# lichunshang/vision-enhanced-lidar-odometry

Measured on AMD Instinct MI355X. Metric: scan-pairs/sec + achieved HBM GB/s, 120k-pt HDL-64E frame-to-frame ICP, higher is better.
Workload: dtype f32 association / f64 residuals+solve

## Files before the change

vision-enhanced-lidar-odometry_amd/csrc/velo_kernels.h:

```cpp
#pragma once
#include <hip/hip_runtime.h>
#include <stdint.h>

#include "velo_device_math.h"

#ifndef VELO_DEF_LOAD
#define VELO_DEF_LOAD 0
#endif
#ifndef VELO_DEF_ASSOC
#define VELO_DEF_ASSOC 0
#endif
#ifndef VELO_DEF_LMA
#define VELO_DEF_LMA 0
#endif
#ifndef VELO_DEF_LMB
#define VELO_DEF_LMB 0
#endif

namespace velo {

constexpr int kWave = 64;
constexpr int kNumAcc = 28;
constexpr int kEvalThreads = 256;
constexpr int kMaxEvalBlocks = 512;
// ... 1042 lines not shown
                        const float d2 = dist2_f(qx, qy, qz, sp.x, sp.y, sp.z);
                        const unsigned long long key = ((unsigned long long)__float_as_uint(d2) << 32) | (unsigned)__float_as_int(sp.w);
                        if (key < b2) {
                            const int ring = G.sring[j];
                            if (key < b1) {
                                if (ring != b1ring) b2 = b1;
                                b1 = key; b1ring = ring;
                            } else if (ring != b1ring) {
                                b2 = key;
                            }
                        }
                    }
                }
            }
        }
    }
    if (active) finish_correspondence(qi, psrc, qx, qy, qz, b1, b2, key_inf, tgt, tgt_off, ring_of, norm_cond, out, want_aux != 0);
}
#else
;
#endif

struct Top2 {
    unsigned long long b1, b2;
    int b1ring, b2ring;
    float b2d;
};
__device__ __forceinline__ void top2_update(Top2& t, unsigned long long key, int ring) {
    if (key < t.b2) {
        if (key < t.b1) {
            if (ring != t.b1ring) { t.b2 = t.b1; t.b2ring = t.b1ring; }
            t.b1 = key; t.b1ring = ring;
        } else if (ring != t.b1ring) {
            t.b2 = key; t.b2ring = ring;
        }
        t.b2d = __uint_as_float((unsigned)(t.b2 >> 32));
    }
}

__device__ __forceinline__ int wave_min_i(int v) {
#pragma unroll
    for (int off = 32; off > 0; off >>= 1) v = min(v, __shfl_xor(v, off));
    return v;
}
__device__ __forceinline__ int wave_max_i(int v) {
#pragma unroll
    for (int off = 32; off > 0; off >>= 1) v = max(v, __shfl_xor(v, off));
    return v;
}

#ifndef VELO_ASSOC_SYNC_LEAN
#define VELO_ASSOC_SYNC_LEAN 1
#endif
constexpr int kTileCap = 512;
typedef float f32x2 __attribute__((ext_vector_type(2)));

template <int NW, int MINW, bool DBG>
__global__ void __launch_bounds__(NW * 64, MINW)
assoc_search_v3_kernel(PoseScalars P, GridView G, const float4* __restrict__ src, const int* __restrict__ q_src, int q_begin, int q_end,
                       const float4* __restrict__ tgt, const int* __restrict__ tgt_off, const int* __restrict__ ring_of,
                       unsigned gate_bits, double norm_cond, int cluster_w, float h_safe, AssocOut out, int want_aux, int dbg, int xcd_map) {
    constexpr int NT = NW * 64;
    constexpr int NRUN = 2 * NT;
    __shared__ float4 s_xy[kTileCap / 2];
    __shared__ float4 s_zg[kTileCap / 2];
    __shared__ int s_ring[kTileCap];
    __shared__ int s_run_j0[NRUN];
    __shared__ int s_run_off[NRUN + 1];
    __shared__ int s_wave_tot[NW];
    __shared__ unsigned long long m1[NW][64], m2[NW][64];
    __shared__ int mr[NW][64];

    const int tid = threadIdx.x;
    const int lane = tid & 63;
    const int wid = __builtin_amdgcn_readfirstlane(tid >> 6);
    long long tacc[8] = {0, 0, 0, 0, 0, 0, 0, 0};
    long long tlast = (DBG && (dbg & 8)) ? (long long)__builtin_readcyclecounter() : 0;
#define VELO_STAMP(k) do { if (DBG && (dbg & 8)) { const long long now__ = (long long)__builtin_readcyclecounter(); tacc[k] += now__ - tlast; tlast = now__; } } while (0)
    const int n_groups = (q_end - q_begin + 63) >> 6;
    const int per_xcd = (n_groups + 7) >> 3;
    const int group = xcd_map ? (int)(blockIdx.x & 7) * per_xcd + (int)(blockIdx.x >> 3) : (int)blockIdx.x;
    if (group >= n_groups || (xcd_map && (int)(blockIdx.x >> 3) >= per_xcd)) return;
    if ((DBG && (dbg & 32)) && threadIdx.x == 0) out.wg_times[2 * group] = __builtin_amdgcn_s_memrealtime();
    const int qi = q_begin + group * 64 + lane;
    const bool active = qi < q_end;
    const unsigned long long key_inf = ((unsigned long long)gate_bits + 1ull) << 32;
    float qx = 0.f, qy = 0.f, qz = 0.f;
    Top2 t;
    t.b1 = key_inf; t.b2 = key_inf; t.b1ring = -1; t.b2ring = -1; t.b2d = __uint_as_float(gate_bits + 1u);
    const GridDesc g = G.d;
    int cx = 0, cy = 0, cz = 0;
    if (active) {
        const float4 psrc = src[q_src[qi]];
        transform_query(P, psrc, &qx, &qy, &qz);
        cx = cell_coord(qx, g.ox, g.inv_h, g.nx); cy = cell_coord(qy, g.oy, g.inv_h, g.ny); cz = cell_coord(qz, g.oz, g.inv_h, g.nz);
    }
    VELO_STAMP(0);
    const f32x2 qx2 = {qx, qx}, qy2 = {qy, qy}, qz2 = {qz, qz};
    float* s_xy_f = reinterpret_cast<float*>(s_xy);
    float* s_zg_f = reinterpret_cast<float*>(s_zg);
    bool pending = active;
    for (;;) {
        const unsigned long long pm = __ballot(pending);
        if (pm == 0ull) break;
        const int leader = (int)__ffsll((long long)pm) - 1;
        const int scx = __builtin_amdgcn_readlane(cx, leader), scy = __builtin_amdgcn_readlane(cy, leader), scz = __builtin_amdgcn_readlane(cz, leader);
// ... 129 lines not shown
                m1[wid][lane] = t.b1; m2[wid][lane] = t.b2; mr[wid][lane] = t.b1ring;
                __syncthreads();
#pragma unroll
                for (int w = 0; w < NW; w++) {
                    if (w == wid) continue;
                    const unsigned long long c1 = m1[w][lane], c2 = m2[w][lane];
                    if (c1 < t.b2) top2_update(t, c1, mr[w][lane]);
                    if (c2 < t.b2) top2_update(t, c2, ring_of[(int)(unsigned)(c2 & 0xffffffffull) - out.first_point]);
                }
                __syncthreads();
            }
            const float rw = __uint_as_float((unsigned)__builtin_amdgcn_readfirstlane(wave_max_i(member ? (int)__float_as_uint(t.b2d) : 0)));
            const float reach = (float)e * h_safe;
            VELO_STAMP(6);
            if (reach * reach > rw) break;
            e_prev = e;
            e = max(e + 1, (int)ceilf(sqrtf(rw) / h_safe));
            if ((float)e * h_safe * ((float)e * h_safe) <= rw) e++;
        }
        pending = pending && !member;
    }
    if (NW > 1 && wid != 0) return;
    if (active) finish_correspondence(qi, src[q_src[qi]], qx, qy, qz, t.b1, t.b2, key_inf, tgt, tgt_off, ring_of, norm_cond, out, want_aux != 0);
    VELO_STAMP(7);
    if ((DBG && (dbg & 32)) && tid == 0) out.wg_times[2 * group + 1] = __builtin_amdgcn_s_memrealtime();
    if ((DBG && (dbg & 8)) && tid == 0) { for (int k = 0; k < 8; k++) atomicAdd((unsigned long long*)&out.dbg[k], (unsigned long long)tacc[k]); }
#undef VELO_STAMP
}

struct CellBox { int x0, x1, y0, y1, z0, z1; };
__device__ __forceinline__ CellBox query_box(const GridDesc& g, float qx, float qy, float qz, int cx, int cy, int cz, float r, bool clip) {
    asm volatile("" : "+v"(r));
    CellBox b;
    b.x0 = cell_coord(qx - r, g.ox, g.inv_h, g.nx); b.x1 = cell_coord(qx + r, g.ox, g.inv_h, g.nx);
    b.y0 = cell_coord(qy - r, g.oy, g.inv_h, g.ny); b.y1 = cell_coord(qy + r, g.oy, g.inv_h, g.ny);
    b.z0 = cell_coord(qz - r, g.oz, g.inv_h, g.nz); b.z1 = cell_coord(qz + r, g.oz, g.inv_h, g.nz);
    if (clip) {
        b.x0 = max(b.x0, cx - 1); b.x1 = min(b.x1, cx + 1);
        b.y0 = max(b.y0, cy - 1); b.y1 = min(b.y1, cy + 1);
        b.z0 = max(b.z0, cz - 1); b.z1 = min(b.z1, cz + 1);
    }
    return b;
}

__device__ __forceinline__ void top2_merge_xor(Top2& t, int mask) {
    const unsigned long long o1 = __shfl_xor(t.b1, mask), o2 = __shfl_xor(t.b2, mask);
    const int r1 = __shfl_xor(t.b1ring, mask), r2 = __shfl_xor(t.b2ring, mask);
    if (o1 < t.b2) top2_update(t, o1, r1);
    if (o2 < t.b2) top2_update(t, o2, r2);
}

#define kXcdChunks (reinterpret_cast<const int*>(8))
#define kXcdTiles (reinterpret_cast<const int*>(16))
template <int NW, int MINW, bool DBG, int PPT, int ASKER>
__device__ __forceinline__ void
assoc_search_v5_body(const PoseScalars& P_in, const PoseRecord* __restrict__ P_dev, int* __restrict__ chain_fail, const GridView& G, const float4* __restrict__ qpts, int q_begin, int q_end,
                     const float4* __restrict__ tgt_pad, const int* __restrict__ tgt_off,
                     unsigned gate_bits, double norm_cond, int cluster_w, float h_safe, const AssocOut& out, int want_aux, const int* __restrict__ group_perm, int dbg, int asker_rows,
                     const int block_x) {
    constexpr int NT = NW * 64;
    constexpr int NRUN = 2 * NT;
    static_assert(kTileCap % (2 * PPT) == 0, "the tile must hold whole trips (the padding of the last trip stays inside it)");
    __shared__ float4 s_xy[kTileCap / 2];
    __shared__ float4 s_zg[kTileCap / 2];
    __shared__ int s_ring[kTileCap];
    __shared__ int s_run_j0[NRUN];
    __shared__ int s_run_off[NRUN + 1];
    __shared__ int s_wave_tot[NW];
    __shared__ int s_lo[NT], s_hi[NT], s_plo[NT], s_phi[NT];
    __shared__ int s_box[2][6][64];
    __shared__ int s_phase[9];
    __shared__ float s_q[3][64];
#define VELO_Q(x, y, z) const float x = s_q[0][lane], y = s_q[1][lane], z = s_q[2][lane]
    static_assert(NW * 64 * 16 <= (int)sizeof(float4) * (kTileCap / 2) && NW * 64 * 8 <= (int)sizeof(int) * kTileCap, "merge scratch must fit the tile");
    unsigned long long (*m1)[64] = reinterpret_cast<unsigned long long (*)[64]>(s_xy);
    unsigned long long (*m2)[64] = m1 + NW;
    int (*mr)[64] = reinterpret_cast<int (*)[64]>(s_ring);
    int (*mr2)[64] = mr + NW;

    const int tid = threadIdx.x;
    const int lane = tid & 63;
    const int wid = __builtin_amdgcn_readfirstlane(tid >> 6);
    constexpr int lead = 0;
    if (chain_fail && *chain_fail) return;
    if (P_dev && !P_dev->ready) { if (block_x == 0 && tid == 0) *chain_fail = 1; return; }
    const PoseScalars& P = P_dev ? P_dev->P : P_in;
    long long tacc[8] = {0, 0, 0, 0, 0, 0, 0, 0};
    long long tlast = (DBG && (dbg & 8)) ? (long long)__builtin_readcyclecounter() : 0;
#define VELO_STAMP(k) do { if (DBG && (dbg & 8)) { const long long now__ = (long long)__builtin_readcyclecounter(); tacc[k] += now__ - tlast; tlast = now__; } } while (0)
    int group = (int)block_x;
    if (group_perm == kXcdChunks) {
        const int n_groups = (q_end - q_begin + 63) / 64, per = (n_groups + 7) / 8;
        group = (block_x & 7) * per + (block_x >> 3);
        if (group >= n_groups) return;
    } else if (group_perm == kXcdTiles) {
        const int n_groups = (q_end - q_begin + 63) / 64, per = (n_groups + 63) / 64;
        const int k = block_x & 7, j = block_x >> 3, b = j / per, w = j - b * per;
        group = (b * 8 + ((k + 8 - (b & 7)) & 7)) * per + w;
        if (b >= 8 || group >= n_groups) return;
    } else if (group_perm) group = group_perm[block_x];
    if (out.n_valid_next && block_x == 0 && tid == 0) *out.n_valid_next = 0;
    if (ASKER == 2 && block_x == 0 && tid == 0) *out.ask_count_next = 0;
    if (DBG && out.wg_times && tid == 0) out.wg_times[2 * group] = __builtin_amdgcn_s_memrealtime();
    const int qi = q_begin + group * 64 + lane;
    const bool active = qi < q_end;
    const unsigned long long key_inf = ((unsigned long long)gate_bits + 1ull) << 32;
    Top2 t;
    t.b1 = key_inf; t.b2 = key_inf; t.b1ring = -1; t.b2ring = -1; t.b2d = __uint_as_float(gate_bits + 1u);
    const GridDesc g = G.d;
#if VELO_ASSOC_SYNC_LEAN
    {
        float qx = 0.f, qy = 0.f, qz = 0.f;
        if (active) {
            const float4 psrc = qpts[qi];
            const bool seeded = out.prev_a && !(DBG && (dbg & 512));
            float4 sa = make_float4(0.f, 0.f, 0.f, __int_as_float(-1)), sb = sa;
            int2 sr = make_int2(-1, -1);
            if (seeded) { sa = out.prev_a[qi]; sb = out.prev_b[qi]; sr = out.prev_r[qi]; }
            transform_query(P, psrc, &qx, &qy, &qz);
            if (__float_as_int(sa.w) >= 0) {
                const float d = dist2_f(sa.x, sa.y, sa.z, qx, qy, qz);
                if (__float_as_uint(d) <= gate_bits) top2_update(t, ((unsigned long long)__float_as_uint(d) << 32) | (unsigned)(__float_as_int(sa.w) + out.first_point), sr.x);
            }
            if (__float_as_int(sb.w) >= 0) {
                const float d = dist2_f(sb.x, sb.y, sb.z, qx, qy, qz);
                if (__float_as_uint(d) <= gate_bits) top2_update(t, ((unsigned long long)__float_as_uint(d) << 32) | (unsigned)(__float_as_int(sb.w) + out.first_point), sr.y);
            }
        }
        s_q[0][lane] = qx; s_q[1][lane] = qy; s_q[2][lane] = qz;
        s_lo[tid] = 1 << 28; s_hi[tid] = -(1 << 28); s_plo[tid] = 1 << 28; s_phi[tid] = -(1 << 28);
    }
#else
    {
        unsigned long long* sb = reinterpret_cast<unsigned long long*>(s_zg);
        int* sr = s_ring;
        if (wid == lead) {
            float qx = 0.f, qy = 0.f, qz = 0.f;
            if (active) {
                const float4 psrc = qpts[qi];
                const bool seeded = out.prev_a && !(DBG && (dbg & 512));
                float4 sa = make_float4(0.f, 0.f, 0.f, __int_as_float(-1)), sb = sa;
                int2 sr = make_int2(-1, -1);
                if (seeded) { sa = out.prev_a[qi]; sb = out.prev_b[qi]; sr = out.prev_r[qi]; }
                transform_query(P, psrc, &qx, &qy, &qz);
                if (__float_as_int(sa.w) >= 0) {
                    const float d = dist2_f(sa.x, sa.y, sa.z, qx, qy, qz);
                    if (__float_as_uint(d) <= gate_bits) top2_update(t, ((unsigned long long)__float_as_uint(d) << 32) | (unsigned)(__float_as_int(sa.w) + out.first_point), sr.x);
                }
                if (__float_as_int(sb.w) >= 0) {
                    const float d = dist2_f(sb.x, sb.y, sb.z, qx, qy, qz);
                    if (__float_as_uint(d) <= gate_bits) top2_update(t, ((unsigned long long)__float_as_uint(d) << 32) | (unsigned)(__float_as_int(sb.w) + out.first_point), sr.y);
                }
            }
            s_q[0][lane] = qx; s_q[1][lane] = qy; s_q[2][lane] = qz;
            sb[lane] = t.b1; sb[64 + lane] = t.b2; sr[lane] = t.b1ring; sr[64 + lane] = t.b2ring;
        }
        __syncthreads();
        if (wid != lead) {
            t.b1 = sb[lane]; t.b2 = sb[64 + lane]; t.b1ring = sr[lane]; t.b2ring = sr[64 + lane];
            t.b2d = __uint_as_float((unsigned)(t.b2 >> 32));
        }
        __syncthreads();
    }
#endif
    VELO_STAMP(0);
    float* s_xy_f = reinterpret_cast<float*>(s_xy);
    float* s_zg_f = reinterpret_cast<float*>(s_zg);
    const int big = 1 << 28;
    bool pending = active;
    bool deferred = false;
    unsigned long long gstat[6] = {0, 0, 0, 0, 0, 0};
    for (;;) {
        const unsigned long long pm = __ballot(pending);
        if (pm == 0ull) break;
        const int leader = (int)__ffsll((long long)pm) - 1;
        bool member;
        {
            VELO_Q(qx, qy, qz);
            int cx = 0, cy = 0, cz = 0;
            if (active) { cx = cell_coord(qx, g.ox, g.inv_h, g.nx); cy = cell_coord(qy, g.oy, g.inv_h, g.ny); cz = cell_coord(qz, g.oz, g.inv_h, g.nz); }
            const int scx = __builtin_amdgcn_readlane(cx, leader), scy = __builtin_amdgcn_readlane(cy, leader), scz = __builtin_amdgcn_readlane(cz, leader);
            member = pending && abs(cx - scx) <= cluster_w && abs(cy - scy) <= cluster_w && abs(cz - scz) <= cluster_w;
        }
        if (DBG && (dbg & 16) && tid == 0) atomicAdd(&out.dbg[0], 1ull);
        if (DBG && (dbg & 32)) gstat[0]++;
        const float r1 = sqrtf(t.b2d) * 1.0001f + 1e-6f;
        bool asker_phase = false;
        const int dense_rows = (ASKER && !DBG) ? (dbg & 0xfffff) : 0, dense_far = (ASKER && !DBG) ? (dbg >> 20) : 0;
        bool asker_all = false;
        for (int ph = 0; ph < 2; ph++) {
            if (ph == 1 && s_phase[7] == 0) break;
            if (wid == lead) {
                bool asks0 = member;
                CellBox bb;
                int rows_all = 0;
                VELO_Q(qx, qy, qz);
                const int cx = cell_coord(qx, g.ox, g.inv_h, g.nx), cy = cell_coord(qy, g.oy, g.inv_h, g.ny), cz = cell_coord(qz, g.oz, g.inv_h, g.nz);
                if (ph == 0) bb = query_box(g, qx, qy, qz, cx, cy, cz, r1, true);
                else {
                    const float rq = sqrtf(t.b2d) * 1.0001f + 1e-6f;
                    bb = query_box(g, qx, qy, qz, cx, cy, cz, rq, false);
                    asks0 = member && !(bb.x0 >= s_box[0][0][lane] && bb.x1 <= s_box[0][1][lane] && bb.y0 >= s_box[0][2][lane] &&
                                        bb.y1 <= s_box[0][3][lane] && bb.z0 >= s_box[0][4][lane] && bb.z1 <= s_box[0][5][lane]);
                    rows_all = asks0 ? (bb.y1 - bb.y0 + 1) * (bb.z1 - bb.z0 + 1) : 0;
#pragma unroll
                    for (int off = 32; off > 0; off >>= 1) rows_all += __shfl_xor(rows_all, off);
                }
                s_box[ph][0][lane] = bb.x0; s_box[ph][1][lane] = bb.x1; s_box[ph][2][lane] = bb.y0;
                s_box[ph][3][lane] = bb.y1; s_box[ph][4][lane] = bb.z0; s_box[ph][5][lane] = bb.z1;
                const unsigned long long am0 = __ballot(asks0);
                const unsigned long long far0 = (ph == 0) ? __ballot(member && r1 > h_safe) : 1ull;
                const unsigned long long far4 = (ASKER && ph == 0) ? __ballot(member && r1 > 4.0f * h_safe) : 0ull;
                const int y0 = wave_min_i(asks0 ? bb.y0 : big), y1 = wave_max_i(asks0 ? bb.y1 : -big);
                const int z0 = wave_min_i(asks0 ? bb.z0 : big), z1 = wave_max_i(asks0 ? bb.z1 : -big);
                if (lane == 0) {
                    s_phase[0] = max(y0, 0); s_phase[1] = min(y1, g.ny - 1); s_phase[2] = max(z0, 0); s_phase[3] = min(z1, g.nz - 1);
                    s_phase[4] = (int)(unsigned)(am0 & 0xffffffffull); s_phase[5] = (int)(unsigned)(am0 >> 32); s_phase[6] = rows_all;
                    if (ph == 0) s_phase[7] = (int)__popcll(far0);
                    if (ASKER && ph == 0) s_phase[8] = (int)__popcll(far4);
                }
            }
            __syncthreads();
            if (ASKER && ph == 0 && dense_rows > 0) {
                const int ny0 = s_phase[1] - s_phase[0] + 1, nz0 = s_phase[3] - s_phase[2] + 1;
// ... 92 lines not shown
                if (tid == 0) s_run_off[NRUN] = total;
                __syncthreads();
                VELO_STAMP(2);
                if (DBG && (dbg & 2)) total = 0;
                if (DBG && (dbg & 32)) { gstat[1]++; gstat[2] += (unsigned long long)total; }
                if (DBG && (dbg & 16) && tid == 0) { atomicAdd(&out.dbg[1], 1ull); atomicAdd(&out.dbg[2], (unsigned long long)total); if (ph == 1) atomicAdd(&out.dbg[3], (unsigned long long)total); atomicAdd(&out.dbg[4], (unsigned long long)nrows); }
                for (int tbase = 0; tbase < total; tbase += kTileCap) {
                    const int tn = min(total - tbase, kTileCap);
                    const int tn2 = (tn + 2 * PPT - 1) / (2 * PPT) * (2 * PPT);
                    for (int i = tid; i < tn2; i += NT) {
                        float4 c = make_float4(__builtin_inff(), __builtin_inff(), __builtin_inff(), __int_as_float(0x7fffffff));
                        int cr = 0x7fffffff;
                        if (i < tn) {
                            const int slot = tbase + i;
                            int lo = 0;
#pragma unroll
                            for (int step = NRUN / 2; step > 0; step >>= 1) {
                                if (s_run_off[lo + step] <= slot) lo += step;
                            }
                            const int j = s_run_j0[lo] + (slot - s_run_off[lo]);
                            c = G.sorted[j];
                            cr = G.sring[j];
                        }
                        const int pr = i >> 1, hb = i & 1;
                        s_xy_f[4 * pr + hb] = c.x; s_xy_f[4 * pr + 2 + hb] = c.y;
                        s_zg_f[4 * pr + hb] = c.z; s_zg_f[4 * pr + 2 + hb] = c.w;
                        s_ring[i] = cr;
                    }
                    __syncthreads();
                    VELO_STAMP(3);
                    const int npairs = tn2 >> 1;
                    if (member && !(DBG && (dbg & 1))) {
                        const int2* s_ring2 = reinterpret_cast<const int2*>(s_ring);
                        for (int pi = wid * PPT; pi < npairs; pi += NW * PPT) {
                            float4 a[PPT], bq[PPT];
                            int2 rg[PPT];
#pragma unroll
                            for (int u = 0; u < PPT; u++) { a[u] = s_xy[pi + u]; bq[u] = s_zg[pi + u]; rg[u] = s_ring2[pi + u]; }
                            float d2x[PPT], d2y[PPT];
                            {
                                VELO_Q(qx, qy, qz);
#pragma unroll
                                for (int u = 0; u < PPT; u++) {
                                    d2x[u] = dist2_f(qx, qy, qz, a[u].x, a[u].z, bq[u].x);
                                    d2y[u] = dist2_f(qx, qy, qz, a[u].y, a[u].w, bq[u].y);
                                }
                            }
                            float dmin = fminf(d2x[0], d2y[0]);
#pragma unroll
                            for (int u = 1; u < PPT; u++) dmin = fminf(dmin, fminf(d2x[u], d2y[u]));
                            if (dmin <= t.b2d) {
#pragma unroll
                                for (int u = 0; u < PPT; u++) {
                                    if (d2x[u] <= t.b2d) {
                                        const unsigned long long key = ((unsigned long long)__float_as_uint(d2x[u]) << 32) | (unsigned)__float_as_int(bq[u].z);
                                        top2_update(t, key, rg[u].x);
                                    }
                                    if (d2y[u] <= t.b2d) {
                                        const unsigned long long key = ((unsigned long long)__float_as_uint(d2y[u]) << 32) | (unsigned)__float_as_int(bq[u].w);
                                        top2_update(t, key, rg[u].y);
                                    }
                                }
                            }
                        }
                    }
                    VELO_STAMP(4);
                    __syncthreads();
                    VELO_STAMP(5);
                }
            }
            if (NW > 1) {
                m1[wid][lane] = t.b1; m2[wid][lane] = t.b2; mr[wid][lane] = t.b1ring; mr2[wid][lane] = t.b2ring;
                __syncthreads();
#pragma unroll
                for (int w = 0; w < NW; w++) {
                    if (w == wid) continue;
                    const unsigned long long c1 = m1[w][lane], c2 = m2[w][lane];
                    if (c1 < t.b2) top2_update(t, c1, mr[w][lane]);
                    if (c2 < t.b2) top2_update(t, c2, mr2[w][lane]);
                }
                if (!VELO_ASSOC_SYNC_LEAN || ASKER != 0) __syncthreads();
            }
            VELO_STAMP(6);
        }
        if (ASKER == 2 && asker_phase) {
            VELO_Q(qx, qy, qz);
            const int cx = cell_coord(qx, g.ox, g.inv_h, g.nx), cy = cell_coord(qy, g.oy, g.inv_h, g.ny), cz = cell_coord(qz, g.oz, g.inv_h, g.nz);
            const float rq0 = sqrtf(t.b2d) * 1.0001f + 1e-6f;
            const CellBox b2 = query_box(g, qx, qy, qz, cx, cy, cz, rq0, false);
            const bool asks = member && (asker_all || !(b2.x0 >= s_box[0][0][lane] && b2.x1 <= s_box[0][1][lane] && b2.y0 >= s_box[0][2][lane] &&
                                                        b2.y1 <= s_box[0][3][lane] && b2.z0 >= s_box[0][4][lane] && b2.z1 <= s_box[0][5][lane]));
            if (wid == 0) {
                const unsigned long long am = __ballot(asks);
                int base = 0;
                if (lane == 0 && am != 0ull) base = atomicAdd(out.ask_count, (int)__popcll(am));
                base = __builtin_amdgcn_readfirstlane(base);
                if (asks) {
                    const int q_of_lane = q_begin + group * 64 + lane;
                    out.ask_list[base + (int)__popcll(am & ((1ull << lane) - 1ull))] = q_of_lane;
                    out.ask_keys[2 * (size_t)q_of_lane] = t.b1; out.ask_keys[2 * (size_t)q_of_lane + 1] = t.b2;
                    out.ask_rings[q_of_lane] = make_int2(t.b1ring, t.b2ring);
                }
            }
            deferred = deferred || asks;
        } else if (ASKER == 1 && asker_phase) {
            const float cap = 4.0f * h_safe;
// ... 37 lines not shown
                    const int nrows_a = (on && x0 <= x1 && ny > 0 && nz > 0) ? ny * nz : 0;
                    const float rcp_ny = 1.0f / (float)max(ny, 1);
                    for (int r0 = 0; r0 < nrows_a; r0 += LPA) {
                        const int r = r0 + sl;
                        int j0 = 0, len = 0;
                        if (r < nrows_a) {
                            int zq = (int)((float)r * rcp_ny), yr = r - zq * ny;
                            if (yr < 0) { zq--; yr += ny; } else if (yr >= ny) { zq++; yr -= ny; }
                            const int row = ((z0 + zq) * g.ny + (y0 + yr));
                            j0 = grid_start(G, row, x0); len = grid_start(G, row, x1 + 1) - j0;
                        }
                        int inc = len;
#pragma unroll
                        for (int off = 1; off < LPA; off <<= 1) { const int v = __shfl_up(inc, off, LPA); if (sl >= off) inc += v; }
                        const int total = __shfl(inc, LPA - 1, LPA);
                        w_j0[sl] = j0; w_off[sl] = inc - len;
                        if (sl == 0) w_off[LPA] = total;
                        __builtin_amdgcn_fence(__ATOMIC_RELEASE, "wavefront");
                        __builtin_amdgcn_wave_barrier();
                        __builtin_amdgcn_fence(__ATOMIC_ACQUIRE, "wavefront");
                        if (DBG && (dbg & 32)) gstat[4] += (unsigned long long)total;
                        if (DBG && (dbg & 16) && sl == 0) { atomicAdd(&out.dbg[2], (unsigned long long)total); atomicAdd(&out.dbg[3], (unsigned long long)total); atomicAdd(&out.dbg[4], (unsigned long long)min(LPA, nrows_a - r0)); }
                        for (int slot = sl; slot < total; slot += LPA) {
                            int lo = 0;
#pragma unroll
                            for (int step = LPA / 2; step > 0; step >>= 1) { if (w_off[lo + step] <= slot) lo += step; }
                            const int j = w_j0[lo] + (slot - w_off[lo]);
                            const float4 c = G.sorted[j];
                            const float d = dist2_f(ax, ay, az, c.x, c.y, c.z);
                            if (d <= tl.b2d) top2_update(tl, ((unsigned long long)__float_as_uint(d) << 32) | (unsigned)__float_as_int(c.w), G.sring[j]);
                        }
                        __builtin_amdgcn_fence(__ATOMIC_RELEASE, "wavefront");
                        __builtin_amdgcn_wave_barrier();
                        __builtin_amdgcn_fence(__ATOMIC_ACQUIRE, "wavefront");
                    }
#pragma unroll
                    for (int m = 1; m < LPA; m <<= 1) top2_merge_xor(tl, m);
                    if (on && sl == 0) { m1[0][la] = tl.b1; m2[0][la] = tl.b2; mr[0][la] = tl.b1ring; mr2[0][la] = tl.b2ring; }
                }
                __syncthreads();
                if (asks) {
                    t.b1 = m1[0][lane]; t.b2 = m2[0][lane]; t.b1ring = mr[0][lane]; t.b2ring = mr2[0][lane];
                    t.b2d = __uint_as_float((unsigned)(t.b2 >> 32));
                }
                __syncthreads();
            }
            if (DBG && (dbg & 32)) gstat[5] += __builtin_amdgcn_s_memrealtime() - t_ask0;
            }
            VELO_STAMP(6);
        }
        pending = pending && !member;
        if (VELO_ASSOC_SYNC_LEAN && ASKER == 0 && __ballot(pending) != 0ull) __syncthreads();
    }
    if (NW > 1 && wid != lead) return;
    VELO_Q(qx, qy, qz);
    int lane_fin = lane;
    asm volatile("" : "+v"(lane_fin));
    const int qi_fin = q_begin + group * 64 + lane_fin;
    const bool active_fin = qi_fin < q_end;
#define qi qi_fin
#define active active_fin
    if (DBG && (dbg & 128)) {
        if (active) { out.p[qi] = make_float4(qx, qy, qz, 0.f); out.n[qi] = make_float4((float)(t.b1 >> 32), (float)(t.b2 >> 32), 0.f, 0.f); out.v0[qi] = make_float4(0.f, 0.f, 0.f, 0.f); }
    } else
    if (active && !deferred) finish_correspondence_pad(qi, qpts, qx, qy, qz, t.b1, t.b2, t.b1ring, t.b2ring, key_inf, tgt_pad, tgt_off, norm_cond, out, want_aux != 0);
    VELO_STAMP(7);
    if (DBG && out.wg_times && tid == 0) {
        out.wg_times[2 * group + 1] = __builtin_amdgcn_s_memrealtime();
        const int n_groups = (q_end - q_begin + 63) / 64;
        for (int k = 0; k < 6; k++) out.wg_times[2 * (size_t)n_groups + 14 * (size_t)group + k] = gstat[k];
        for (int k = 0; k < 8; k++) out.wg_times[2 * (size_t)n_groups + 14 * (size_t)group + 6 + k] = (unsigned long long)tacc[k];
    }
    if (DBG && (dbg & 8) && tid == 0) { for (int k = 0; k < 8; k++) atomicAdd((unsigned long long*)&out.dbg[k], (unsigned long long)tacc[k]); }
#undef VELO_STAMP
#undef VELO_Q
#undef qi
#undef active
}


template <int NW, int MINW, bool DBG, int PPT, int ASKER>
__global__ void __launch_bounds__(NW * 64, MINW)
assoc_search_v5_kernel(PoseScalars P, const PoseRecord* __restrict__ P_dev, int* __restrict__ chain_fail, GridView G, const float4* __restrict__ qpts, int q_begin, int q_end,
                       const float4* __restrict__ tgt_pad, const int* __restrict__ tgt_off,
                       unsigned gate_bits, double norm_cond, int cluster_w, float h_safe, AssocOut out, int want_aux, const int* __restrict__ group_perm, int dbg, int asker_rows) {
    assoc_search_v5_body<NW, MINW, DBG, PPT, ASKER>(P, P_dev, chain_fail, G, qpts, q_begin, q_end, tgt_pad, tgt_off, gate_bits, norm_cond, cluster_w, h_safe, out,
                                                    want_aux, group_perm, dbg, asker_rows, (int)blockIdx.x);
}

constexpr int kAssocBatchMax = 4;
struct AssocArgs {
    PoseScalars P; const PoseRecord* P_dev; int* chain_fail; GridView G; const float4* qpts; int q_begin, q_end;
    const float4* tgt_pad; const int* tgt_off; unsigned gate_bits; double norm_cond; int cluster_w; float h_safe;
    AssocOut out; int want_aux; const int* group_perm; int dbg; int asker_rows;
};
struct AssocBatch { AssocArgs item[kAssocBatchMax]; };
template <int NW, int MINW, bool DBG, int PPT, int ASKER>
__global__ void __launch_bounds__(NW * 64, MINW)
assoc_search_v5_batch_kernel(AssocBatch B) {
    const AssocArgs& a = B.item[blockIdx.y];
    if (a.group_perm != kXcdChunks && a.group_perm != kXcdTiles && (int)blockIdx.x * 64 >= a.q_end - a.q_begin) return;
    assoc_search_v5_body<NW, MINW, DBG, PPT, ASKER>(a.P, a.P_dev, a.chain_fail, a.G, a.qpts, a.q_begin, a.q_end, a.tgt_pad, a.tgt_off, a.gate_bits, a.norm_cond,
                                                    a.cluster_w, a.h_safe, a.out, a.want_aux, a.group_perm, a.dbg, a.asker_rows, (int)blockIdx.x);
}

constexpr int kAskChunk = 8;
__device__ __forceinline__ void asker_search(const GridView& G, const GridDesc& g, float ax, float ay, float az, float rq, Top2& tl, int lane,
                                             int* __restrict__ w_j0, int* __restrict__ w_off) {
    const CellBox bb = query_box(g, ax, ay, az, 0, 0, 0, rq, false);
    const int x0 = max(bb.x0, 0), x1 = min(bb.x1, g.nx - 1);
    const int y0 = max(bb.y0, 0), y1 = min(bb.y1, g.ny - 1), z0 = max(bb.z0, 0), z1 = min(bb.z1, g.nz - 1);
    const int ny = y1 - y0 + 1, nz = z1 - z0 + 1;
    const int nrows_a = (x0 <= x1 && ny > 0 && nz > 0) ? ny * nz : 0;
    const float rcp_ny = 1.0f / (float)max(ny, 1);
    for (int r0 = 0; r0 < nrows_a; r0 += 64) {
        const int r = r0 + lane;
        int j0 = 0, len = 0;
        if (r < nrows_a) {
            int zq = (int)((float)r * rcp_ny), yr = r - zq * ny;
            if (yr < 0) { zq--; yr += ny; } else if (yr >= ny) { zq++; yr -= ny; }
            const int row = ((z0 + zq) * g.ny + (y0 + yr));
            j0 = grid_start(G, row, x0); len = grid_start(G, row, x1 + 1) - j0;
        }
        int inc = len;
#pragma unroll
        for (int off = 1; off < 64; off <<= 1) { const int v = __shfl_up(inc, off); if (lane >= off) inc += v; }
        const int total = __shfl(inc, 63);
        w_j0[lane] = j0; w_off[lane] = inc - len;
        __builtin_amdgcn_fence(__ATOMIC_RELEASE, "wavefront");
        __builtin_amdgcn_wave_barrier();
        __builtin_amdgcn_fence(__ATOMIC_ACQUIRE, "wavefront");
        for (int slot = lane; slot < total; slot += 128) {
            const int slot2 = slot + 64;
            const bool two = slot2 < total;
            int lo = 0, lo2 = 0;
#pragma unroll
            for (int step = 32; step > 0; step >>= 1) {
                if (w_off[lo + step] <= slot) lo += step;
                if (w_off[lo2 + step] <= slot2) lo2 += step;
            }
            const int j = w_j0[lo] + (slot - w_off[lo]);
            const int j2 = two ? w_j0[lo2] + (slot2 - w_off[lo2]) : j;
            const float4 c = G.sorted[j], c2 = G.sorted[j2];
            const float d = dist2_f(ax, ay, az, c.x, c.y, c.z), d2 = dist2_f(ax, ay, az, c2.x, c2.y, c2.z);
            if (d <= tl.b2d) top2_update(tl, ((unsigned long long)__float_as_uint(d) << 32) | (unsigned)__float_as_int(c.w), G.sring[j]);
            if (two && d2 <= tl.b2d) top2_update(tl, ((unsigned long long)__float_as_uint(d2) << 32) | (unsigned)__float_as_int(c2.w), G.sring[j2]);
        }
        __builtin_amdgcn_fence(__ATOMIC_RELEASE, "wavefront");
        __builtin_amdgcn_wave_barrier();
        __builtin_amdgcn_fence(__ATOMIC_ACQUIRE, "wavefront");
    }
#pragma unroll
    for (int m = 1; m < 64; m <<= 1) top2_merge_xor(tl, m);
}

// ... 2447 lines not shown
        const double m[3] = {-x[0], -x[1], -x[2]};
        pose_rot_init(m, &s_Rinv);
        s_t[0] = x[3]; s_t[1] = x[4]; s_t[2] = x[5];
    }
    __syncthreads();
    const int i = blockIdx.x * blockDim.x + threadIdx.x;
    if (i >= n) return;
    const FunctorRec F = f[i];
    const double t[3] = {s_t[0], s_t[1], s_t[2]};
    double r[3] = {0.0, 0.0, 0.0}, J[18];
#pragma unroll
    for (int k = 0; k < 18; k++) J[k] = 0.0;
    switch (F.kind) {
        case 0: res_3d3d(s_R, t, F.c, F.c + 3, r, J); break;
        case 1: res_3d2d(s_R, t, F.c, F.c + 3, F.c + 5, r, J); break;
        case 2: res_2d3d(s_Rinv, t, F.c, F.c + 3, F.c + 5, r, J); break;
        case 3: res_2d2d(s_R, t, F.c, F.c + 2, F.c + 4, r, J); break;
        default: res_3dpd(s_R, t, F.c, F.c + 3, F.c + 6, r, J); break;
    }
#pragma unroll
    for (int k = 0; k < 3; k++) res[(size_t)3 * i + k] = r[k];
    if (jac) {
#pragma unroll
        for (int k = 0; k < 18; k++) jac[(size_t)18 * i + k] = J[k];
    }
}
#else
;
#endif

#ifndef VELO_UNIT_LM_ONLY
#if VELO_DEF_LOAD
#define VELO_INST_LOAD template
#else
#define VELO_INST_LOAD extern template
#endif
#if VELO_DEF_ASSOC
#define VELO_INST_ASSOC template
#else
#define VELO_INST_ASSOC extern template
#endif
VELO_INST_LOAD __global__ void scan_lookback_kernel<kLbItemsSmall>(int*, int, unsigned long long*, int*, int*);
VELO_INST_LOAD __global__ void scan_lookback_kernel<kLbItemsLarge>(int*, int, unsigned long long*, int*, int*);
VELO_INST_LOAD __global__ void advance_scan_kernel<kLbItemsSmall>(AdvBatch);
VELO_INST_LOAD __global__ void advance_scan_kernel<kLbItemsLarge>(AdvBatch);
#define VELO_V5_ARGS (PoseScalars, const PoseRecord*, int*, GridView, const float4*, int, int, const float4*, const int*, unsigned, double, int, float, AssocOut, int, const int*, int, int)
#define VELO_V3_ARGS (PoseScalars, GridView, const float4*, const int*, int, int, const float4*, const int*, const int*, unsigned, double, int, float, AssocOut, int, int, int)
#define VELO_CLUSTER_ARGS (GridView, AssocQueue, const float4*, const int*, int, int, const float4*, const int*, const int*, unsigned, double, float, AssocOut, int)
VELO_INST_ASSOC __global__ void assoc_search_v5_kernel<4, 5, false, 2, 0> VELO_V5_ARGS;
VELO_INST_ASSOC __global__ void assoc_search_v5_kernel<4, 5, false, 2, 1> VELO_V5_ARGS;
VELO_INST_ASSOC __global__ void assoc_search_v5_batch_kernel<4, 5, false, 2, 0>(AssocBatch);
VELO_INST_ASSOC __global__ void assoc_search_v5_batch_kernel<4, 5, false, 2, 1>(AssocBatch);
VELO_INST_ASSOC __global__ void assoc_search_v5_batch_kernel<4, 5, false, 2, 2>(AssocBatch);
#ifdef VELO_DIAGNOSTICS
VELO_INST_ASSOC __global__ void assoc_search_v5_kernel<4, 5, true, 2, 1> VELO_V5_ARGS;
VELO_INST_ASSOC __global__ void assoc_search_v5_kernel<4, 5, false, 4, 1> VELO_V5_ARGS;
VELO_INST_ASSOC __global__ void assoc_search_v5_kernel<4, 6, false, 2, 1> VELO_V5_ARGS;
VELO_INST_ASSOC __global__ void assoc_search_v5_kernel<4, 6, false, 2, 0> VELO_V5_ARGS;
VELO_INST_ASSOC __global__ void assoc_search_v5_kernel<4, 7, false, 2, 0> VELO_V5_ARGS;
VELO_INST_ASSOC __global__ void assoc_search_v5_kernel<4, 8, false, 2, 0> VELO_V5_ARGS;
VELO_INST_ASSOC __global__ void assoc_search_v3_kernel<1, 1, false> VELO_V3_ARGS;
VELO_INST_ASSOC __global__ void assoc_search_v3_kernel<1, 1, true> VELO_V3_ARGS;
VELO_INST_ASSOC __global__ void assoc_search_v3_kernel<2, 1, false> VELO_V3_ARGS;
VELO_INST_ASSOC __global__ void assoc_search_v3_kernel<2, 1, true> VELO_V3_ARGS;
VELO_INST_ASSOC __global__ void assoc_search_v3_kernel<4, 5, false> VELO_V3_ARGS;
VELO_INST_ASSOC __global__ void assoc_search_v3_kernel<4, 5, true> VELO_V3_ARGS;
VELO_INST_ASSOC __global__ void assoc_search_v3_kernel<4, 6, false> VELO_V3_ARGS;
VELO_INST_ASSOC __global__ void assoc_search_v3_kernel<4, 6, true> VELO_V3_ARGS;
VELO_INST_ASSOC __global__ void assoc_search_v3_kernel<4, 7, false> VELO_V3_ARGS;
VELO_INST_ASSOC __global__ void assoc_search_v3_kernel<4, 7, true> VELO_V3_ARGS;
VELO_INST_ASSOC __global__ void assoc_search_v3_kernel<4, 8, false> VELO_V3_ARGS;
VELO_INST_ASSOC __global__ void assoc_search_v3_kernel<4, 8, true> VELO_V3_ARGS;
VELO_INST_ASSOC __global__ void assoc_search_v3_kernel<8, 8, false> VELO_V3_ARGS;
VELO_INST_ASSOC __global__ void assoc_search_v3_kernel<8, 8, true> VELO_V3_ARGS;
VELO_INST_ASSOC __global__ void assoc_cluster_kernel<2, 1> VELO_CLUSTER_ARGS;
VELO_INST_ASSOC __global__ void assoc_cluster_kernel<4, 6> VELO_CLUSTER_ARGS;
VELO_INST_ASSOC __global__ void assoc_cluster_kernel<8, 6> VELO_CLUSTER_ARGS;
#endif
#undef VELO_V5_ARGS
#undef VELO_V3_ARGS
#undef VELO_CLUSTER_ARGS
#endif

}
```

Measured before the change: 4335.

## Let one assoc workgroup process several query groups and add strict top2 filter

Adds a GPW template parameter so one 4-wave workgroup handles several 64-query groups in sequence. Each group's query transform and seeded top-2 are parked in LDS and its final result is written back by a dedicated wave. A STRICT variant gates top2 updates behind a wave ballot that skips updates no lane needs. New instantiations are compiled only when the macros differ from GPW=1/STRICT=0; the default macro sets STRICT=1, which instantiates a <...,1,true> kernel, but whether the host launches it is not shown.

```diff
diff --git a/vision-enhanced-lidar-odometry_amd/csrc/velo_kernels.h b/vision-enhanced-lidar-odometry_amd/csrc/velo_kernels.h
--- a/vision-enhanced-lidar-odometry_amd/csrc/velo_kernels.h
+++ b/vision-enhanced-lidar-odometry_amd/csrc/velo_kernels.h
@@ -1118,6 +1118,15 @@
 #ifndef VELO_ASSOC_SYNC_LEAN
 #define VELO_ASSOC_SYNC_LEAN 1
 #endif
+#ifndef VELO_ASSOC_GPW
+#define VELO_ASSOC_GPW 1
+#endif
+#ifndef VELO_ASSOC_STRICT
+#define VELO_ASSOC_STRICT 1
+#endif
+constexpr int kAssocGpw = VELO_ASSOC_GPW;
+constexpr bool kAssocStrict = VELO_ASSOC_STRICT != 0;
+constexpr int assoc_gpw_lds(int gpw) { return gpw > 1 ? gpw * 64 * 24 + (gpw - 1) * 64 * 12 : 0; }
 constexpr int kTileCap = 512;
 typedef float f32x2 __attribute__((ext_vector_type(2)));
 
@@ -1353,7 +1362,7 @@
 
 #define kXcdChunks (reinterpret_cast<const int*>(8))
 #define kXcdTiles (reinterpret_cast<const int*>(16))
-template <int NW, int MINW, bool DBG, int PPT, int ASKER>
+template <int NW, int MINW, bool DBG, int PPT, int ASKER, int GPW = 1, bool STRICT = false>
 __device__ __forceinline__ void
 assoc_search_v5_body(const PoseScalars& P_in, const PoseRecord* __restrict__ P_dev, int* __restrict__ chain_fail, const GridView& G, const float4* __restrict__ qpts, int q_begin, int q_end,
                      const float4* __restrict__ tgt_pad, const int* __restrict__ tgt_off,
@@ -1371,8 +1380,13 @@
     __shared__ int s_lo[NT], s_hi[NT], s_plo[NT], s_phi[NT];
     __shared__ int s_box[2][6][64];
     __shared__ int s_phase[9];
-    __shared__ float s_q[3][64];
-#define VELO_Q(x, y, z) const float x = s_q[0][lane], y = s_q[1][lane], z = s_q[2][lane]
+    static_assert(GPW >= 1 && GPW <= NW, "one wave per group sets up and finishes");
+    static_assert(GPW == 1 || (ASKER == 0 && !DBG && VELO_ASSOC_SYNC_LEAN), "several groups per workgroup: regular-grid product instantiation only");
+    __shared__ float s_q[GPW][3][64];
+    __shared__ unsigned long long s_park[GPW > 1 ? GPW : 1][2][64];
+    __shared__ int s_park_ring[GPW > 1 ? GPW : 1][2][64];
+    int gslot = 0;
+#define VELO_Q(x, y, z) const float x = s_q[gslot][0][lane], y = s_q[gslot][1][lane], z = s_q[gslot][2][lane]
     static_assert(NW * 64 * 16 <= (int)sizeof(float4) * (kTileCap / 2) && NW * 64 * 8 <= (int)sizeof(int) * kTileCap, "merge scratch must fit the tile");
     unsigned long long (*m1)[64] = reinterpret_cast<unsigned long long (*)[64]>(s_xy);
     unsigned long long (*m2)[64] = m1 + NW;
@@ -1389,8 +1403,23 @@
     long long tacc[8] = {0, 0, 0, 0, 0, 0, 0, 0};
     long long tlast = (DBG && (dbg & 8)) ? (long long)__builtin_readcyclecounter() : 0;
 #define VELO_STAMP(k) do { if (DBG && (dbg & 8)) { const long long now__ = (long long)__builtin_readcyclecounter(); tacc[k] += now__ - tlast; tlast = now__; } } while (0)
+    auto slot_group = [&](int s) -> int {
+        const int n_groups = (q_end - q_begin + 63) / 64;
+        int gq = s;
+        if (group_perm == kXcdChunks) {
+            const int per = (n_groups + 7) / 8;
+            gq = (s >> 3) < per ? (s & 7) * per + (s >> 3) : -1;
+        } else if (group_perm == kXcdTiles) {
+            const int per = (n_groups + 63) / 64;
+            const int k = s & 7, j = s >> 3, b = j / max(per, 1), w = j - b * per;
+            gq = (b * 8 + ((k + 8 - (b & 7)) & 7)) * per + w;
+            if (b >= 8) gq = -1;
+        } else if (group_perm) gq = s < n_groups ? group_perm[s] : -1;
+        return (gq >= 0 && gq < n_groups) ? gq : -1;
+    };
     int group = (int)block_x;
-    if (group_perm == kXcdChunks) {
+    if (GPW > 1) group = slot_group(block_x * GPW);
+    else if (group_perm == kXcdChunks) {
         const int n_groups = (q_end - q_begin + 63) / 64, per = (n_groups + 7) / 8;
         group = (block_x & 7) * per + (block_x >> 3);
         if (group >= n_groups) return;
@@ -1403,12 +1432,38 @@
     if (out.n_valid_next && block_x == 0 && tid == 0) *out.n_valid_next = 0;
     if (ASKER == 2 && block_x == 0 && tid == 0) *out.ask_count_next = 0;
     if (DBG && out.wg_times && tid == 0) out.wg_times[2 * group] = __builtin_amdgcn_s_memrealtime();
-    const int qi = q_begin + group * 64 + lane;
-    const bool active = qi < q_end;
+    int qi = q_begin + group * 64 + lane;
+    bool active = (GPW == 1 || group >= 0) && qi < q_end;
     const unsigned long long key_inf = ((unsigned long long)gate_bits + 1ull) << 32;
     Top2 t;
     t.b1 = key_inf; t.b2 = key_inf; t.b1ring = -1; t.b2ring = -1; t.b2d = __uint_as_float(gate_bits + 1u);
     const GridDesc g = G.d;
+    if (GPW > 1) {
+        if (wid < GPW) {
+            const int gw = slot_group(block_x * GPW + wid);
+            const int qw = q_begin + gw * 64 + lane;
+            float qx = 0.f, qy = 0.f, qz = 0.f;
+            if (gw >= 0 && qw < q_end) {
+                const float4 psrc = qpts[qw];
+                float4 sa = make_float4(0.f, 0.f, 0.f, __int_as_float(-1)), sb = sa;
+                int2 sr = make_int2(-1, -1);
+                if (out.prev_a) { sa = out.prev_a[qw]; sb = out.prev_b[qw]; sr = out.prev_r[qw]; }
+                transform_query(P, psrc, &qx, &qy, &qz);
+                if (__float_as_int(sa.w) >= 0) {
+                    const float d = dist2_f(sa.x, sa.y, sa.z, qx, qy, qz);
+                    if (__float_as_uint(d) <= gate_bits) top2_update(t, ((unsigned long long)__float_as_uint(d) << 32) | (unsigned)(__float_as_int(sa.w) + out.first_point), sr.x);
+                }
+                if (__float_as_int(sb.w) >= 0) {
+                    const float d = dist2_f(sb.x, sb.y, sb.z, qx, qy, qz);
+                    if (__float_as_uint(d) <= gate_bits) top2_update(t, ((unsigned long long)__float_as_uint(d) << 32) | (unsigned)(__float_as_int(sb.w) + out.first_point), sr.y);
+                }
+            }
+            s_q[wid][0][lane] = qx; s_q[wid][1][lane] = qy; s_q[wid][2][lane] = qz;
+            s_park[wid][0][lane] = t.b1; s_park[wid][1][lane] = t.b2; s_park_ring[wid][0][lane] = t.b1ring; s_park_ring[wid][1][lane] = t.b2ring;
+        }
+        s_lo[tid] = 1 << 28; s_hi[tid] = -(1 << 28); s_plo[tid] = 1 << 28; s_phi[tid] = -(1 << 28);
+        __syncthreads();
+    } else
 #if VELO_ASSOC_SYNC_LEAN
     {
         float qx = 0.f, qy = 0.f, qz = 0.f;
@@ -1428,7 +1483,7 @@
                 if (__float_as_uint(d) <= gate_bits) top2_update(t, ((unsigned long long)__float_as_uint(d) << 32) | (unsigned)(__float_as_int(sb.w) + out.first_point), sr.y);
             }
         }
-        s_q[0][lane] = qx; s_q[1][lane] = qy; s_q[2][lane] = qz;
+        s_q[0][0][lane] = qx; s_q[0][1][lane] = qy; s_q[0][2][lane] = qz;
         s_lo[tid] = 1 << 28; s_hi[tid] = -(1 << 28); s_plo[tid] = 1 << 28; s_phi[tid] = -(1 << 28);
     }
 #else
@@ -1453,7 +1508,7 @@
                     if (__float_as_uint(d) <= gate_bits) top2_update(t, ((unsigned long long)__float_as_uint(d) << 32) | (unsigned)(__float_as_int(sb.w) + out.first_point), sr.y);
                 }
             }
-            s_q[0][lane] = qx; s_q[1][lane] = qy; s_q[2][lane] = qz;
+            s_q[0][0][lane] = qx; s_q[0][1][lane] = qy; s_q[0][2][lane] = qz;
             sb[lane] = t.b1; sb[64 + lane] = t.b2; sr[lane] = t.b1ring; sr[64 + lane] = t.b2ring;
         }
         __syncthreads();
@@ -1471,6 +1526,16 @@
     bool pending = active;
     bool deferred = false;
     unsigned long long gstat[6] = {0, 0, 0, 0, 0, 0};
+#pragma unroll 1
+    for (gslot = 0; gslot < GPW; gslot++) {
+    if (GPW > 1) {
+        group = slot_group(block_x * GPW + gslot);
+        qi = q_begin + group * 64 + lane;
+        active = group >= 0 && qi < q_end;
+        t.b1 = s_park[gslot][0][lane]; t.b2 = s_park[gslot][1][lane]; t.b1ring = s_park_ring[gslot][0][lane]; t.b2ring = s_park_ring[gslot][1][lane];
+        t.b2d = __uint_as_float((unsigned)(t.b2 >> 32));
+        pending = active;
+    }
     for (;;) {
         const unsigned long long pm = __ballot(pending);
         if (pm == 0ull) break;
@@ -1669,6 +1734,17 @@
                             if (dmin <= t.b2d) {
 #pragma unroll
                                 for (int u = 0; u < PPT; u++) {
+                                    if (STRICT) {
+                                        if (d2x[u] <= t.b2d) {
+                                            const unsigned long long key = ((unsigned long long)__float_as_uint(d2x[u]) << 32) | (unsigned)__float_as_int(bq[u].z);
+                                            if (key < t.b2 && __builtin_amdgcn_ballot_w64(key < t.b1 || rg[u].x != t.b1ring) != 0ull) top2_update(t, key, rg[u].x);
+                                        }
+                                        if (d2y[u] <= t.b2d) {
+                                            const unsigned long long key = ((unsigned long long)__float_as_uint(d2y[u]) << 32) | (unsigned)__float_as_int(bq[u].w);
+                                            if (key < t.b2 && __builtin_amdgcn_ballot_w64(key < t.b1 || rg[u].y != t.b1ring) != 0ull) top2_update(t, key, rg[u].y);
+                                        }
+                                        continue;
+                                    }
                                     if (d2x[u] <= t.b2d) {
                                         const unsigned long long key = ((unsigned long long)__float_as_uint(d2x[u]) << 32) | (unsigned)__float_as_int(bq[u].z);
                                         top2_update(t, key, rg[u].x);
@@ -1812,7 +1888,21 @@
         pending = pending && !member;
         if (VELO_ASSOC_SYNC_LEAN && ASKER == 0 && __ballot(pending) != 0ull) __syncthreads();
     }
-    if (NW > 1 && wid != lead) return;
+    if (GPW > 1) {
+        if (wid == gslot) { s_park[gslot][0][lane] = t.b1; s_park[gslot][1][lane] = t.b2; s_park_ring[gslot][0][lane] = t.b1ring; s_park_ring[gslot][1][lane] = t.b2ring; }
+        if (gslot + 1 < GPW) __syncthreads();
+    }
+    }
+    if (GPW > 1) {
+        if (wid >= GPW) return;
+        gslot = wid;
+        group = slot_group(block_x * GPW + wid);
+        if (group < 0) return;
+        t.b1 = s_park[wid][0][lane]; t.b2 = s_park[wid][1][lane]; t.b1ring = s_park_ring[wid][0][lane]; t.b2ring = s_park_ring[wid][1][lane];
+    } else {
+        gslot = 0;
+        if (NW > 1 && wid != lead) return;
+    }
     VELO_Q(qx, qy, qz);
     int lane_fin = lane;
     asm volatile("" : "+v"(lane_fin));
@@ -1839,12 +1929,12 @@
 }
 
 
-template <int NW, int MINW, bool DBG, int PPT, int ASKER>
+template <int NW, int MINW, bool DBG, int PPT, int ASKER, int GPW = 1, bool STRICT = false>
 __global__ void __launch_bounds__(NW * 64, MINW)
 assoc_search_v5_kernel(PoseScalars P, const PoseRecord* __restrict__ P_dev, int* __restrict__ chain_fail, GridView G, const float4* __restrict__ qpts, int q_begin, int q_end,
                        const float4* __restrict__ tgt_pad, const int* __restrict__ tgt_off,
                        unsigned gate_bits, double norm_cond, int cluster_w, float h_safe, AssocOut out, int want_aux, const int* __restrict__ group_perm, int dbg, int asker_rows) {
-    assoc_search_v5_body<NW, MINW, DBG, PPT, ASKER>(P, P_dev, chain_fail, G, qpts, q_begin, q_end, tgt_pad, tgt_off, gate_bits, norm_cond, cluster_w, h_safe, out,
+    assoc_search_v5_body<NW, MINW, DBG, PPT, ASKER, GPW, STRICT>(P, P_dev, chain_fail, G, qpts, q_begin, q_end, tgt_pad, tgt_off, gate_bits, norm_cond, cluster_w, h_safe, out,
                                                     want_aux, group_perm, dbg, asker_rows, (int)blockIdx.x);
 }
 
@@ -1855,12 +1945,12 @@
     AssocOut out; int want_aux; const int* group_perm; int dbg; int asker_rows;
 };
 struct AssocBatch { AssocArgs item[kAssocBatchMax]; };
-template <int NW, int MINW, bool DBG, int PPT, int ASKER>
+template <int NW, int MINW, bool DBG, int PPT, int ASKER, int GPW = 1, bool STRICT = false>
 __global__ void __launch_bounds__(NW * 64, MINW)
 assoc_search_v5_batch_kernel(AssocBatch B) {
     const AssocArgs& a = B.item[blockIdx.y];
-    if (a.group_perm != kXcdChunks && a.group_perm != kXcdTiles && (int)blockIdx.x * 64 >= a.q_end - a.q_begin) return;
-    assoc_search_v5_body<NW, MINW, DBG, PPT, ASKER>(a.P, a.P_dev, a.chain_fail, a.G, a.qpts, a.q_begin, a.q_end, a.tgt_pad, a.tgt_off, a.gate_bits, a.norm_cond,
+    if (a.group_perm != kXcdChunks && a.group_perm != kXcdTiles && (int)blockIdx.x * GPW * 64 >= a.q_end - a.q_begin) return;
+    assoc_search_v5_body<NW, MINW, DBG, PPT, ASKER, GPW, STRICT>(a.P, a.P_dev, a.chain_fail, a.G, a.qpts, a.q_begin, a.q_end, a.tgt_pad, a.tgt_off, a.gate_bits, a.norm_cond,
                                                     a.cluster_w, a.h_safe, a.out, a.want_aux, a.group_perm, a.dbg, a.asker_rows, (int)blockIdx.x);
 }
 
@@ -4414,6 +4504,21 @@
 VELO_INST_ASSOC __global__ void assoc_search_v5_batch_kernel<4, 5, false, 2, 0>(AssocBatch);
 VELO_INST_ASSOC __global__ void assoc_search_v5_batch_kernel<4, 5, false, 2, 1>(AssocBatch);
 VELO_INST_ASSOC __global__ void assoc_search_v5_batch_kernel<4, 5, false, 2, 2>(AssocBatch);
+#define VELO_INST_V5_GROUPS(GPW, STRICT)                                                                        \
+    VELO_INST_ASSOC __global__ void assoc_search_v5_kernel<4, 5, false, 2, 0, GPW, STRICT> VELO_V5_ARGS;       \
+    VELO_INST_ASSOC __global__ void assoc_search_v5_batch_kernel<4, 5, false, 2, 0, GPW, STRICT>(AssocBatch);
+#ifndef VELO_DIAGNOSTICS
+#if VELO_ASSOC_GPW != 1 || VELO_ASSOC_STRICT != 0
+VELO_INST_V5_GROUPS(kAssocGpw, kAssocStrict)
+#endif
+#else
+VELO_INST_V5_GROUPS(1, true)
+VELO_INST_V5_GROUPS(2, false)
+VELO_INST_V5_GROUPS(2, true)
+VELO_INST_V5_GROUPS(4, false)
+VELO_INST_V5_GROUPS(4, true)
+#endif
+#undef VELO_INST_V5_GROUPS
 #ifdef VELO_DIAGNOSTICS
 VELO_INST_ASSOC __global__ void assoc_search_v5_kernel<4, 5, true, 2, 1> VELO_V5_ARGS;
 VELO_INST_ASSOC __global__ void assoc_search_v5_kernel<4, 5, false, 4, 1> VELO_V5_ARGS;
```

After: 4382 (median of 6 runs). +1.1%, better.
